# MattJBorowski1991/QuantizedMHA

Hardware: AMD Instinct MI355X
Metric: attention-fwd TFLOPS + ms/call, B16 H16 N4096 d64 (fp16 & int8) (higher is better)
Workload: dtype int8; 1 GPU; fa_tc_int8_b attention forward (BASELINE config 4); variant=fa_tc_int8_b, B_per_gpu=16, H=16, N=4096, d=64, d_model=1024, global_batch=16, parallelism=batch-shard x1 (no collective in the timed step; all-gather reported separately)

## Files before the change

quantizedmha_amd/csrc/qmha_fa_int8.hip:

```cpp
#include "qmha_common.hpp"
#include "qmha_kernels.hpp"

#include <atomic>
#include <type_traits>

namespace qmha {

static constexpr float kPtSumCap = 2047.0f / 127.0f;

template <int D>
__device__ __forceinline__ float quant_q_operand(const float* __restrict__ row, int half, v4i (&qop)[D / 32],
                                                 float slice_sc = 0.0f) {
    constexpr int KS = D / 32;
    v4f x[KS][4];
    float amax = 0.0f;
#pragma unroll
    for (int s = 0; s < KS; ++s)
#pragma unroll
        for (int c4 = 0; c4 < 4; ++c4) {
            x[s][c4] = *reinterpret_cast<const v4f*>(row + 32 * s + 16 * half + 4 * c4);
#pragma unroll
            for (int e = 0; e < 4; ++e) {
                x[s][c4][e] = nan_to_zero(x[s][c4][e]);
                amax = fmaxf(amax, fabsf(x[s][c4][e]));
            }
        }
    const float sc = slice_sc > 0.0f ? slice_sc : qmha_scale_from_absmax(wave_max64(amax));
    const float inv = 1.0f / sc;
#pragma unroll
    for (int s = 0; s < KS; ++s)
#pragma unroll
        for (int c4 = 0; c4 < 4; ++c4) {
            uint32_t w = 0;
#pragma unroll
            for (int e = 0; e < 4; ++e) w |= ((uint32_t)(uint8_t)qmha_quant_i8(x[s][c4][e], inv)) << (8 * e);
            qop[s][c4] = (int)w;
        }
    return sc;
}

__device__ PDump g_pdump;

enum { FL_MAGIC = 1, FL_LB1 = 2, FL_LB2 = 4, FL_JIT = 8, FL_LB4 = 16, FL_KFOLD = 64, FL_DUMP = 256, FL_PT = 1048576 };

template <int D, int FL>
__global__ __launch_bounds__(256, (FL & FL_LB1) ? 1 : ((FL & FL_LB2) ? 2 : 4)) void qmha_fa_int8_kernel(
    const float* __restrict__ Qf, const int8_t* __restrict__ Ki, const _Float16* __restrict__ Vh,
    const float* __restrict__ sK, const float* __restrict__ sV,
    float* __restrict__ O, int N, int H, int d_model, int nqb, float c_log2, QkDump dbg) {
    constexpr int WAVES = 4, SG = 2;
    constexpr int KS = D / 32;
    constexpr int KBYTES = SG * 32 * D;
    constexpr int VBYTES = SG * 32 * D * 2;
    constexpr int KCH = KBYTES / 16, VCH = VBYTES / 16;
    constexpr bool MAGIC = FL & FL_MAGIC;
    constexpr bool DUMP = FL & FL_DUMP;
    static_assert(D % 32 == 0 && D <= 256, "d % 32 == 0 (include/config.h:32), d <= 256 (MAGIC range)");
    static_assert(KCH % 64 == 0 && VCH % 64 == 0, "a stage is whole KiB LDS-DMA pieces");
    static_assert((KCH / SG) % 64 == 0, "a KV group is whole KiB pieces (D >= 32)");
    __shared__ __attribute__((aligned(16))) int8_t lds[2][KBYTES + VBYTES];

    const int G = N / QMHA_GROUP;
    const int wg = xcd_remap(blockIdx.x, gridDim.x);
    const int bh = wg / nqb, qb = wg % nqb;
    const int b = bh / H, k = bh % H;
    const int lane = threadIdx.x & 63;
    const int wave = __builtin_amdgcn_readfirstlane(threadIdx.x >> 6);
    const int half = lane >> 5, col = lane & 31;
    const int qg = qb * WAVES + wave;
    const bool active = qg < G;

    PDump pd{};
    if constexpr (DUMP) pd = g_pdump;
    size_t drow = 0;
    if constexpr (DUMP) drow = (size_t)bh * N + (size_t)qg * QMHA_GROUP + col;
    v4i qop[KS];
    float cq = 0.0f;
    if (active) {
        const float* qrow = Qf + ((size_t)b * N + (size_t)qg * QMHA_GROUP + col) * d_model + (size_t)k * D;
        const float sq = quant_q_operand<D>(qrow, half, qop);
        cq = sq * c_log2;
        if constexpr (DUMP) {
            int8_t* qd = dbg.Qi + ((size_t)bh * N + (size_t)qg * QMHA_GROUP + col) * D + 16 * half;
#pragma unroll
            for (int s = 0; s < KS; ++s) *reinterpret_cast<v4i*>(qd + 32 * s) = qop[s];
            if (lane == 0) dbg.sQ[(size_t)bh * G + qg] = sq;
        }
    } else {
#pragma unroll
        for (int s = 0; s < KS; ++s) qop[s] = v4i{0, 0, 0, 0};
    }
    v16f o[KS];
#pragma unroll
    for (int m = 0; m < KS; ++m) o[m] = v16f{};
    float m_run = 0.0f;
    float l_run = 0.0f;
    float anchor = 0.0f;

    const int8_t* kbase = Ki + (size_t)bh * N * D;
    const char* vbase = reinterpret_cast<const char*>(Vh + (size_t)bh * N * D);
    const float* skb = sK + (size_t)bh * G;
    const float* svb = sV + (size_t)bh * G;
    const int nst = (G + SG - 1) / SG;

    auto issue = [&](int buf, int st) {
        const int ngr = min(SG, G - st * SG);
        const int8_t* ksrc = kbase + (size_t)st * KBYTES;
        const char* vsrc = vbase + (size_t)st * VBYTES;
        int8_t* L = lds[buf];
#pragma unroll
        for (int jj = 0; jj < (KCH / 64 + WAVES - 1) / WAVES; ++jj) {
            const int inst = wave + jj * WAVES;
            if (inst < KCH / 64 && inst * 64 < ngr * (KCH / SG)) {
                const int idx = inst * 64 + lane;
                const int row = idx / (D / 16), cc = swz_src<D>(row, idx % (D / 16));
                __builtin_amdgcn_global_load_lds((gptr_t)(ksrc + row * D + 16 * cc), (lptr_t)(L + inst * 1024), 16, 0, 0);
            }
        }
#pragma unroll
        for (int jj = 0; jj < (VCH / 64 + WAVES - 1) / WAVES; ++jj) {
            const int inst = wave + jj * WAVES;
            if (inst < VCH / 64 && inst * 64 < ngr * (VCH / SG)) {
                const int idx = inst * 64 + lane;
                const int grp = idx / (4 * D), w = idx % (4 * D);
                const int d = w >> 2, cv = swz_src<64>(d, w & 3);
                __builtin_amdgcn_global_load_lds((gptr_t)(vsrc + grp * 64 * D + d * 64 + 16 * cv),
// ... 67 lines not shown
        const float e = __builtin_amdgcn_exp2f(m_new - anchor);
        l_run = fmaf(rs, e, l_run);
        m_run = m_new;
        const float scale = sp * svt * e;
#pragma unroll
        for (int m = 0; m < KS; ++m) {
            const int d = 32 * m + col;
            const int8_t* vr = L + KBYTES + gi * 64 * D + d * 64;
            v16f acc = v16f{};
#pragma unroll
            for (int ks = 0; ks < 2; ++ks) {
                const v8h vop = *reinterpret_cast<const v8h*>(vr + 16 * swz_pos<64>(d, 2 * ks + half));
                acc = __builtin_amdgcn_mfma_f32_32x32x16_f16(vop, pop[ks], acc, 0, 0, 0);
            }
            if constexpr (DUMP) {
                if (active && pd.m)
                    dump_pv_acc<false>(pd.T + (((size_t)bh * G + t) * N + qg * QMHA_GROUP + col) * D + 32 * m, acc, half);
            }
#pragma unroll
            for (int r = 0; r < 16; ++r) o[m][r] = fmaf(acc[r], scale, o[m][r]);
        }
    };

    issue(0, 0);
    qmha_dma_barrier();

    for (int st = 0; st < nst; ++st) {
        const int buf = st & 1;
        if (st + 1 < nst) issue(buf ^ 1, st + 1);
        if (active) {
            const int g0 = st * SG;
            const int ngr = min(SG, G - g0);
            const int8_t* L = lds[buf];
            if (ngr == SG) {
#pragma unroll
                for (int gi = 0; gi < SG; ++gi) tile(L, gi, g0 + gi, qk(L, gi));
            } else {
                for (int gi = 0; gi < ngr; ++gi) tile(L, gi, g0 + gi, qk(L, gi));
            }
        }
        qmha_dma_barrier();
    }

    if (active) {
        const float unanchor = __builtin_amdgcn_exp2f(anchor - m_run);
        const float l = l_run * unanchor;
        if constexpr (DUMP) {
            if (pd.m && half == 0) pd.l[drow] = l;
        }
        const bool ok = l > 1e-20f;
        float* orow = O + ((size_t)b * N + (size_t)qg * QMHA_GROUP + col) * d_model + (size_t)k * D + 4 * half;
#pragma unroll
        for (int m = 0; m < KS; ++m)
#pragma unroll
            for (int g4 = 0; g4 < 4; ++g4) {
                v4f w;
#pragma unroll
                for (int jj = 0; jj < 4; ++jj) w[jj] = ok ? (o[m][4 * g4 + jj] * unanchor) / l : 0.0f;
                *reinterpret_cast<v4f*>(orow + 32 * m + 8 * g4) = w;
            }
    }
}

__host__ __device__ constexpr int pt_slot_op(int D, int s, int j) {
    constexpr int d32[6][2] = {{0, -1}, {-1, -1}, {1, -1}, {8, -1}, {-1, -1}, {-1, -1}};
    constexpr int d64[6][2] = {{0, -1}, {2, -1}, {1, -1}, {8, -1}, {9, -1}, {3, -1}};
    constexpr int d128[6][2] = {{0, 2}, {4, 6}, {1, 3}, {8, 9}, {10, 11}, {5, 7}};
    return D == 32 ? d32[s][j] : D == 64 ? d64[s][j] : d128[s][j];
}

template <int N>
__device__ __forceinline__ void pin_regs(float (&v)[N], int lo, int hi) {
#pragma unroll
    for (int i = 0; i < N; ++i)
        if (i >= lo && i < hi) asm volatile("" : "+v"(v[i]));
}

template <int D, int WAVES, int FL>
__global__ __launch_bounds__(WAVES * 64, (FL & FL_LB2) ? 2 : ((FL & FL_LB4) ? 4 : 3)) void qmha_fa_int8_pipe_kernel(
    const float* __restrict__ Qf, const int8_t* __restrict__ Ki, const _Float16* __restrict__ Vh,
    const float* __restrict__ sK, const float* __restrict__ sV,
    float* __restrict__ O, int N, int H, int d_model, int nqb, float c_log2, QkDump dbg,
    const float* __restrict__ sQt = nullptr, int fair = 0) {
    constexpr int SG = 2, RING = 3, PF = RING - 1;
    constexpr int KBYTES = SG * 32 * D;
    constexpr int VBYTES = SG * 32 * D * 2;
    constexpr int SBYTES = KBYTES + VBYTES;
    constexpr int KCH = KBYTES / 16, VCH = VBYTES / 16;
    constexpr bool MAGIC = FL & FL_MAGIC;
    __shared__ __attribute__((aligned(16))) int8_t lds[RING][SBYTES];

    const int G = N / QMHA_GROUP;
    const int wg = xcd_remap(blockIdx.x, gridDim.x);
    const int bh = wg / nqb, qb = wg % nqb;
    const int b = bh / H, k = bh % H;
    const int lane = threadIdx.x & 63;
    const int wave = __builtin_amdgcn_readfirstlane(threadIdx.x >> 6);
    const int half = lane >> 5, col = lane & 31;
    const int qg = qb * WAVES + wave;
    const bool active = qg < G;

    v4i qop[D / 32];
    float cq = 0.0f;
    constexpr bool DUMP = FL & FL_DUMP;
    constexpr bool PT = FL & FL_PT;
    PDump pd{};
    size_t drow = 0;
    if constexpr (DUMP && !PT) {
        pd = g_pdump;
        drow = (size_t)bh * N + (size_t)qg * QMHA_GROUP + col;
    }
    auto dump_t = [&](int t, const v16f (&acc)[D / 32]) {
        if (active && pd.m) {
#pragma unroll
            for (int m = 0; m < D / 32; ++m)
                dump_pv_acc<true>(pd.T + (((size_t)bh * G + t) * N + qg * QMHA_GROUP + col) * D + 32 * m, acc[m], half);
        }
    };
    if (active) {
        const float* qrow = Qf + ((size_t)b * N + (size_t)qg * QMHA_GROUP + col) * d_model + (size_t)k * D;
        const float sq = quant_q_operand<D>(qrow, half, qop, PT ? sQt[bh] : 0.0f);
        cq = sq * c_log2;
        if constexpr (DUMP) {
            int8_t* qd = dbg.Qi + ((size_t)bh * N + (size_t)qg * QMHA_GROUP + col) * D + 16 * half;
#pragma unroll
            for (int s = 0; s < D / 32; ++s) *reinterpret_cast<v4i*>(qd + 32 * s) = qop[s];
            if (lane == 0) dbg.sQ[(size_t)bh * G + qg] = sq;
        }
    } else {
#pragma unroll
        for (int ks = 0; ks < D / 32; ++ks) qop[ks] = v4i{0, 0, 0, 0};
    }
    const int8_t* kbase = Ki + (size_t)bh * N * D;
    const char* vbase = reinterpret_cast<const char*>(Vh) + (size_t)bh * N * D * 2;
    const int sstride = PT ? 1 : G;
    const float* skb = sK + (size_t)bh * sstride;
    const float* svb = sV + (size_t)bh * sstride;
    const int nst = (G + SG - 1) / SG;

    constexpr int KJ = (KCH / 64 + WAVES - 1) / WAVES, VJ = (VCH / 64 + WAVES - 1) / WAVES;
    constexpr bool SPREAD = WAVES >= KCH / 64 + VCH / 64;
    const int vw = SPREAD ? (wave + WAVES - KCH / 64) % WAVES : wave;
    int koff[KJ], voff[VJ];
#pragma unroll
    for (int jj = 0; jj < KJ; ++jj) {
        const int idx = (wave + jj * WAVES) * 64 + lane;
        const int row = idx / (D / 16), cc = swz_src<D>(row, idx % (D / 16));
        koff[jj] = row * D + 16 * cc;
    }
#pragma unroll
    for (int jj = 0; jj < VJ; ++jj) {
        const int idx = (vw + jj * WAVES) * 64 + lane;
        const int grp = idx / (4 * D), w = idx % (4 * D);
        const int d = w >> 2, cv = swz_src<64>(d, w & 3);
        voff[jj] = grp * 64 * D + d * 64 + 16 * cv;
    }
    auto issue_at = [&](int st, int slot) {
        const int ngr = min(SG, G - st * SG);
        int8_t* L = lds[slot];
#pragma unroll
        for (int jj = 0; jj < KJ; ++jj) {
            const int inst = wave + jj * WAVES;
            if (inst < KCH / 64 && inst * 64 < ngr * (KCH / SG))
                buffer_load_lds16(kbase, N * D, (lptr_t)(L + inst * 1024), koff[jj], st * KBYTES);
        }
#pragma unroll
        for (int jj = 0; jj < VJ; ++jj) {
            const int inst = vw + jj * WAVES;
            if (inst < VCH / 64 && inst * 64 < ngr * (VCH / SG))
                buffer_load_lds16(vbase, N * D * 2, (lptr_t)(L + KBYTES + inst * 1024), voff[jj], st * VBYTES);
        }
    };
    auto issue = [&](int st) { issue_at(st, st % RING); };
    auto kop_at = [&](int slot, int par, int ks) {
        const int8_t* L = lds[slot];
        const int krow = par * 32 + col;
        return *reinterpret_cast<const v4i*>(L + krow * D + 16 * swz_pos<D>(krow, 2 * ks + half));
    };
    auto vop_at = [&](int slot, int par, int m, int ks) {
        const int8_t* L = lds[slot];
        const int d = 32 * m + col;
        return *reinterpret_cast<const v8h*>(L + KBYTES + par * 64 * D + d * 64 + 16 * swz_pos<64>(d, 2 * ks + half));
    };
    auto kop_of = [&](int t, int ks) { return kop_at((t >> 1) % RING, t & 1, ks); };
    auto vop_of = [&](int t, int m, int ks) { return vop_at((t >> 1) % RING, t & 1, m, ks); };

    v16i magic_blk;
#pragma unroll
    for (int r = 0; r < 16; ++r) magic_blk[r] = MAGIC ? 0x4B400000 : 0;
    if constexpr (MAGIC) asm volatile("" : "+v"(magic_blk));

    constexpr int MB = D / 32;
    constexpr int KS = D / 32;
    constexpr int NOPS = 2 * MB + KS;
    constexpr int kSlot64[6] = {1, 1, 1, 1, 1, 1};
    constexpr int kOps64[6] = {0, 2, 1, 1000, 3, 1001};
    constexpr int kSlot32[6] = {1, 0, 1, 1, 0, 0};
    constexpr int kOps32[3] = {0, 1, 1000};
    constexpr int kSlot128[6] = {2, 2, 2, 2, 2, 2};
    constexpr int kOps128[12] = {0, 2, 4, 1000, 6, 1, 1001, 3, 5, 1002, 7, 1003};
    auto slot_n = [&](int c) { return D == 32 ? kSlot32[c] : (D == 64 ? kSlot64[c] : kSlot128[c]); };
    auto op_at = [&](int i) { return D == 32 ? kOps32[i] : (D == 64 ? kOps64[i] : kOps128[i]); };
    static_assert(D == 32 || D == 64 || D == 128, "pipelined kernel: d in {32, 64, 128}");
    static_assert(NOPS == (D == 32 ? 3 : (D == 64 ? 6 : 12)), "MFMA schedule table");

    v16f o[MB];
#pragma unroll
    for (int m = 0; m < MB; ++m) o[m] = v16f{};
    float m_run = 0.0f;
    float l_run = 0.0f;
    float anchor = 0.0f;
    v16i s_cur, s_nxt;
    auto qk = [&](const v4i& kk, int ks) {
        s_nxt = __builtin_amdgcn_mfma_i32_32x32x32_i8(kk, qop[ks], ks == 0 ? magic_blk : s_nxt, 0, 0, 0);
    };
    v8h pc[2], pp[2];
    float scale_prev = 0.0f;
    v16f a[MB];
    constexpr bool JIT = FL & FL_JIT;
    constexpr bool KFOLD = MAGIC && (FL & FL_KFOLD);
    static_assert(KFOLD, "the pipelined kernel ships with FL_MAGIC | FL_KFOLD");
    float h_c = 0.0f, h_m = 0.0f, h_k = 0.0f, h_f = 1.0f, h_sp = 0.0f, h_invp = 0.0f, h_cap = 0.0f;
    const float c_pt = PT ? __int_as_float((__float_as_int(cq * skb[0]) + 2) & ~3) : 0.0f;
    auto head = [&](const v16i& s, int t) {
        float c = PT ? c_pt : cq * skb[t];
        const int mxi = half_swap_max_i(tree_max16_i(s));
        if constexpr (!PT) c = __int_as_float((__float_as_int(c) + 2) & ~3);
        const float sfmax = __int_as_float(mxi) - QMHA_MAGIC_RNE;
        const float xm = sfmax * c;
        h_m = fmaxf(m_run, xm);
        h_k = fmaf(c, QMHA_MAGIC_RNE, h_m);
        const float delta = fmaf(c, -QMHA_MAGIC_RNE, h_k) - h_m;
        h_f = fmaf(delta, 0.69314718055994531f, 1.0f);
        const float xmax = fmaf(sfmax, c, -h_m);
        h_c = c;
        const float pmax = half_max32_nonneg(__builtin_amdgcn_exp2f(xmax));
        const float sp = fmaxf(pmax, 1.27e-6f) * (1.0f / 127.0f);
        h_invp = __builtin_amdgcn_rcpf(sp);
        h_invp *= h_f;
        h_sp = sp * 16777216.0f;
    };

    auto pt_base = [&](float mb) {
        h_m = mb;
        h_k = fmaf(c_pt, QMHA_MAGIC_RNE, mb);
        const float delta = fmaf(c_pt, -QMHA_MAGIC_RNE, h_k) - mb;
        h_f = fmaf(delta, 0.69314718055994531f, 1.0f);
        h_invp = 127.0f * h_f;
        h_cap = kPtSumCap / h_f;
    };
    auto pt_rowmax = [&](const v16i& s) {
        return (__int_as_float(half_swap_max_i(tree_max16_i(s))) - QMHA_MAGIC_RNE) * c_pt;
    };
    if constexpr (PT) pt_base(0.0f);
    issue(0);
    if (nst > 1) issue(1);
    qmha_dma_barrier();
#pragma unroll
    for (int ks = 0; ks < KS; ++ks) qk(kop_of(0, ks), ks);
    s_cur = s_nxt;

#define QMHA_FENCE() __builtin_amdgcn_sched_barrier(0)
    auto iter = [&](int t, auto HP, auto HN, auto PH) {
        constexpr bool has_prev = decltype(HP)::value, has_next = decltype(HN)::value;
        constexpr int ph = decltype(PH)::value;
        const int odd = ph >= 0 ? ((1 + ph) & 1) : (t & 1);
        const int slot_p = ph >= 0 ? ((ph >> 1) % RING) : (((t - 1) >> 1) % RING);
        const int par_p = ph >= 0 ? (ph & 1) : ((t - 1) & 1);
        const int slot_nx = ph >= 0 ? (((2 + ph) >> 1) % RING) : (((t + 1) >> 1) % RING);
        const int par_n = ph >= 0 ? (ph & 1) : ((t + 1) & 1);
        auto vop = [&](int m, int ks) { return vop_at(slot_p, par_p, m, ks); };
        auto kop = [&](int ks) { return kop_at(slot_nx, par_n, ks); };
        const int dma_st = (t >> 1) + PF;
        const int dma_slot = ph >= 0 ? ((((1 + ph) >> 1) + PF) % RING) : (((t >> 1) + PF) % RING);
        if (odd) {
            qmha_dma_barrier();
            if (dma_st < nst) issue_at(dma_st, dma_slot);
        }
        if constexpr (DUMP) {
            if (active) {
                int32_t* sd = dbg.S + ((size_t)bh * N + (size_t)qg * QMHA_GROUP + col) * N + (size_t)t * QMHA_GROUP;
#pragma unroll
                for (int r = 0; r < 16; ++r) sd[acc_row(r, half)] = s_cur[r] - 0x4B400000;
            }
        }
        v8h vv[MB][2];
        v4i kk[KS];
        if constexpr (has_prev && !JIT) {
#pragma unroll
            for (int ks = 0; ks < 2; ++ks)
#pragma unroll
                for (int m = 0; m < MB; ++m) vv[m][ks] = vop(m, ks);
        }
        if constexpr (has_next && !JIT) {
#pragma unroll
            for (int ks = 0; ks < KS; ++ks) kk[ks] = kop(ks);
        }
        QMHA_FENCE();
        int op_i = 0;
        auto mfmas = [&](int c) {
#pragma unroll
            for (int j = 0; j < 2; ++j) {
                if (j < slot_n(c)) {
                    const int op = op_at(op_i++);
                    if (op >= 1000) {
                        const int ks = op - 1000;
                        if (has_next) qk(JIT ? kop(ks) : kk[ks], ks);
                    } else {
                        const int m = op >> 1, ks = op & 1;
                        if (has_prev)
                            a[m] = __builtin_amdgcn_mfma_f32_32x32x16_f16(JIT ? vop(m, ks) : vv[m][ks], pp[ks],
                                                                          ks == 0 ? v16f{} : a[m], 0, 0, 0);
                    }
                }
            }
        };
        head(s_cur, t);
        QMHA_FENCE();
        const float c = h_c, m_new = h_m, kn = h_k;
        if (__builtin_amdgcn_ballot_w64(m_new - anchor > 48.0f)) {
            const float f = __builtin_amdgcn_exp2f(anchor - m_new);
#pragma unroll
            for (int m = 0; m < MB; ++m) o[m] *= f;
            l_run *= f;
            scale_prev *= f;
            anchor = m_new;
        }
        mfmas(0);
        QMHA_FENCE();
        const float sp = h_sp, invp = h_invp;
        const float e = __builtin_amdgcn_exp2f(m_new - anchor);
        float x[16];
#pragma unroll
        for (int r = 0; r < 8; ++r) x[r] = fmaf(__int_as_float(s_cur[r]), c, -kn);
        QMHA_FENCE();
        mfmas(1);
        QMHA_FENCE();
#pragma unroll
        for (int r = 8; r < 16; ++r) x[r] = fmaf(__int_as_float(s_cur[r]), c, -kn);
        QMHA_FENCE();
        mfmas(2);
        QMHA_FENCE();
        float p[16];
#pragma unroll
        for (int r = 0; r < 8; ++r) p[r] = __builtin_amdgcn_exp2f(x[r]);
        QMHA_FENCE();
        mfmas(3);
        QMHA_FENCE();
#pragma unroll
        for (int r = 8; r < 16; ++r) p[r] = __builtin_amdgcn_exp2f(x[r]);
        QMHA_FENCE();
        mfmas(4);
        QMHA_FENCE();
#pragma unroll
        for (int r = 0; r < 8; ++r) {
            const float t0 = fmaf(p[2 * r], invp, QMHA_MAGIC_RNE), t1 = fmaf(p[2 * r + 1], invp, QMHA_MAGIC_RNE);
            const v2h h2 = __builtin_bit_cast(v2h, __builtin_amdgcn_perm(__float_as_uint(t1), __float_as_uint(t0), 0x05040100u));
            pc[r >> 2][2 * (r & 3)] = h2[0];
            pc[r >> 2][2 * (r & 3) + 1] = h2[1];
        }
        if constexpr (DUMP) {
            if (active && pd.m) {
                if (half == 0) pd.m[drow * G + t] = m_new;
                if (lane == 0) pd.sP[((size_t)bh * G + qg) * G + t] = sp * (1.0f / 16777216.0f);
                dump_p_operand<true>(pd.Pi + drow * N + (size_t)t * QMHA_GROUP, pc, half);
            }
        }
        QMHA_FENCE();
        mfmas(5);
        QMHA_FENCE();
        const float rs = tree_sum16(p);
        l_run = fmaf(rs, e * h_f, l_run);
        m_run = m_new;
        const float scale_t = sp * svb[t] * e;
        if constexpr (has_prev) {
            if constexpr (DUMP) dump_t(t - 1, a);
#pragma unroll
            for (int m = 0; m < MB; ++m)
#pragma unroll
                for (int r = 0; r < 16; ++r) o[m][r] = fmaf(a[m][r], scale_prev, o[m][r]);
        }
        QMHA_FENCE();
        pp[0] = pc[0];
        pp[1] = pc[1];
        scale_prev = scale_t;
        if constexpr (has_next) s_cur = s_nxt;
    };
    float alpha_prev = 1.0f;
    bool rescale_prev = false;
    auto iter_pt = [&](int t, auto HP, auto HN, auto PH) {
        constexpr bool has_prev = decltype(HP)::value, has_next = decltype(HN)::value;
        constexpr int ph = decltype(PH)::value;
        const int odd = ph >= 0 ? ((1 + ph) & 1) : (t & 1);
        const int slot_p = ph >= 0 ? ((ph >> 1) % RING) : (((t - 1) >> 1) % RING);
        const int par_p = ph >= 0 ? (ph & 1) : ((t - 1) & 1);
        const int slot_nx = ph >= 0 ? (((2 + ph) >> 1) % RING) : (((t + 1) >> 1) % RING);
        const int par_n = ph >= 0 ? (ph & 1) : ((t + 1) & 1);
        const int dma_st = (t >> 1) + PF;
        const int dma_slot = ph >= 0 ? ((((1 + ph) >> 1) + PF) % RING) : (((t >> 1) + PF) % RING);
        if (odd) {
            qmha_dma_barrier();
            if (dma_st < nst) issue_at(dma_st, dma_slot);
        }
        if constexpr (DUMP) {
            if (active) {
                int32_t* sd = dbg.S + ((size_t)bh * N + (size_t)qg * QMHA_GROUP + col) * N + (size_t)t * QMHA_GROUP;
#pragma unroll
                for (int r = 0; r < 16; ++r) sd[acc_row(r, half)] = s_cur[r] - 0x4B400000;
            }
        }
        v8h vv[MB][2];
        v4i kk[KS];
        auto rd_slot = [&](int s) {
#pragma unroll
            for (int j = 0; j < 2; ++j) {
                const int op = pt_slot_op(D, s, j);
                if (op >= 0 && op < 8) {
                    if constexpr (has_prev)
                        if ((op >> 1) < MB) vv[(op >> 1) % MB][op & 1] = vop_at(slot_p, par_p, op >> 1, op & 1);
                } else if (op >= 8) {
                    if constexpr (has_next)
                        if (op - 8 < KS) kk[(op - 8) % KS] = kop_at(slot_nx, par_n, op - 8);
                }
            }
        };
        auto mf_slot = [&](int s) {
#pragma unroll
            for (int j = 0; j < 2; ++j) {
                const int op = pt_slot_op(D, s, j);
                if (op >= 0 && op < 8) {
                    if constexpr (has_prev) {
                        const int m = (op >> 1) % MB;
                        if ((op >> 1) < MB) o[m] = __builtin_amdgcn_mfma_f32_32x32x16_f16(vv[m][op & 1], pp[op & 1], o[m], 0, 0, 0);
                    }
                } else if (op >= 8) {
                    if constexpr (has_next)
                        if (op - 8 < KS) qk(kk[(op - 8) % KS], op - 8);
                }
            }
        };
        float x[16], p[16], q[16];
        auto exps = [&](int r0, int r1) {
#pragma unroll
            for (int r = 0; r < 16; ++r)
                if (r >= r0 && r < r1) p[r] = __builtin_amdgcn_exp2f(x[r]);
        };
        auto quant = [&](int r0, int r1) {
#pragma unroll
            for (int r = 0; r < 16; ++r)
                if (r >= r0 && r < r1) q[r] = fmaf(p[r], h_invp, QMHA_MAGIC_RNE);
        };
        auto perms = [&](int j0, int j1) {
#pragma unroll
            for (int j = 0; j < 8; ++j)
                if (j >= j0 && j < j1) {
                    const v2h h2 = __builtin_bit_cast(v2h, __builtin_amdgcn_perm(__float_as_uint(q[2 * j + 1]),
                                                                               __float_as_uint(q[2 * j]), 0x05040100u));
// ... 45 lines not shown
        QMHA_FENCE();
        mf_slot(2);
        QMHA_FENCE();
        exps(8, 12);
        perms(2, 4);
        QMHA_FENCE();
        rd_slot(4);
        quant(8, 12);
        float rs2 = (p[8] + p[9]) + (p[10] + p[11]);
        asm volatile("" : "+v"(rs2));
        QMHA_FENCE();
        mf_slot(3);
        QMHA_FENCE();
        exps(12, 16);
        perms(4, 6);
        QMHA_FENCE();
        rd_slot(5);
        quant(12, 16);
        float rs3 = (p[12] + p[13]) + (p[14] + p[15]);
        asm volatile("" : "+v"(rs3));
        QMHA_FENCE();
        mf_slot(4);
        QMHA_FENCE();
        perms(6, 8);
        QMHA_FENCE();
        float ts = (rs0 + rs1) + (rs2 + rs3);
        float alpha_t = 1.0f;
        bool rescale_t = false;
        if constexpr (has_prev) {
            const uint64_t over = __builtin_amdgcn_ballot_w64(ts > h_cap);
            if (over) {
                rescale_t = true;
                const float xm = pt_rowmax(s_cur);
                const uint32_t rows = (uint32_t)over | (uint32_t)(over >> 32);
                const float mb = ((rows >> col) & 1u) ? xm : m_run;
                alpha_t = __builtin_amdgcn_exp2f(m_run - mb);
                l_run *= alpha_t;
                pt_base(mb);
                m_run = mb;
#pragma unroll
                for (int r = 0; r < 16; ++r) x[r] = fmaf(__int_as_float(s_cur[r]), c_pt, -h_k);
                exps(0, 16);
                quant(0, 16);
                perms(0, 8);
                ts = tree_sum16(p);
            }
        }
        l_run = fmaf(ts, h_f, l_run);
        QMHA_FENCE();
        mf_slot(5);
        QMHA_FENCE();
        pp[0] = pc[0];
        pp[1] = pc[1];
        alpha_prev = alpha_t;
        rescale_prev = rescale_t;
        if constexpr (has_next) s_cur = s_nxt;
    };
    auto run_iter = [&](int t, auto HP, auto HN, auto PH) {
        if constexpr (PT)
            iter_pt(t, HP, HN, PH);
        else
            iter(t, HP, HN, PH);
    };
    using T1 = std::integral_constant<bool, true>;
    using F0 = std::integral_constant<bool, false>;
    using DYN = std::integral_constant<int, -1>;
    if (PT && G == 1) {
        if constexpr (PT) run_iter(0, F0{}, F0{}, DYN{});
    } else {
        auto set_prio = [&](int tt) {
            const int q = (4 * tt) / G;
            if (q <= 0)
                __builtin_amdgcn_s_setprio(3);
            else if (q == 1)
                __builtin_amdgcn_s_setprio(2);
            else if (q == 2)
                __builtin_amdgcn_s_setprio(1);
            else
                __builtin_amdgcn_s_setprio(0);
        };
        if (fair) set_prio(0);
        run_iter(0, F0{}, T1{}, DYN{});
        int t = 1;
        constexpr int PER = 2 * RING;
        for (; t + PER <= G - 1; t += PER) {
            if (fair) set_prio(t);
            run_iter(t, T1{}, T1{}, std::integral_constant<int, 0>{});
            run_iter(t + 1, T1{}, T1{}, std::integral_constant<int, 1>{});
            run_iter(t + 2, T1{}, T1{}, std::integral_constant<int, 2>{});
            run_iter(t + 3, T1{}, T1{}, std::integral_constant<int, 3>{});
            run_iter(t + 4, T1{}, T1{}, std::integral_constant<int, 4>{});
            run_iter(t + 5, T1{}, T1{}, std::integral_constant<int, 5>{});
        }
        for (; t < G - 1; ++t) run_iter(t, T1{}, T1{}, DYN{});
        run_iter(G - 1, T1{}, F0{}, DYN{});
    }
#undef QMHA_FENCE
    {
        const int t = G - 1;
        if constexpr (PT) {
            if (rescale_prev) {
#pragma unroll
                for (int m = 0; m < MB; ++m) o[m] *= alpha_prev;
            }
#pragma unroll
            for (int ks = 0; ks < 2; ++ks)
#pragma unroll
                for (int m = 0; m < MB; ++m)
                    o[m] = __builtin_amdgcn_mfma_f32_32x32x16_f16(vop_of(t, m, ks), pp[ks], o[m], 0, 0, 0);
        } else {
#pragma unroll
            for (int ks = 0; ks < 2; ++ks)
#pragma unroll
                for (int m = 0; m < MB; ++m)
                    a[m] = __builtin_amdgcn_mfma_f32_32x32x16_f16(vop_of(t, m, ks), pp[ks], ks == 0 ? v16f{} : a[m], 0, 0, 0);
            if constexpr (DUMP) dump_t(t, a);
#pragma unroll
            for (int m = 0; m < MB; ++m) o[m] += a[m] * scale_prev;
        }
    }
    if (active) {
        const float unanchor = PT ? 16777216.0f * (svb[0] / 127.0f) : __builtin_amdgcn_exp2f(anchor - m_run);
        const float l = PT ? half_swap_add(l_run) : half_swap_add(l_run) * unanchor;
        if constexpr (DUMP && !PT) {
            if (pd.m && half == 0) pd.l[drow] = l;
        }
        const bool ok = l > 1e-20f;
        float* orow = O + ((size_t)b * N + (size_t)qg * QMHA_GROUP + col) * d_model + (size_t)k * D + 4 * half;
#pragma unroll
        for (int m = 0; m < MB; ++m)
#pragma unroll
            for (int g4 = 0; g4 < 4; ++g4) {
                v4f w;
#pragma unroll
                for (int jj = 0; jj < 4; ++jj) w[jj] = ok ? (o[m][4 * g4 + jj] * unanchor) / l : 0.0f;
                *reinterpret_cast<v4f*>(orow + 32 * m + 8 * g4) = w;
            }
    }
}

template <int D>
__global__ __launch_bounds__(64) void qmha_debug_qk_int32_kernel(const int8_t* __restrict__ Qi, const int8_t* __restrict__ Ki,
                                                                int N, int bh, int32_t* __restrict__ S) {
    constexpr int KS = D / 32;
    const int qg = blockIdx.x, kg = blockIdx.y;
    const int lane = threadIdx.x, half = lane >> 5, col = lane & 31;
    const int8_t* qp = Qi + ((size_t)bh * N + (size_t)qg * 32 + col) * D + 16 * half;
    const int8_t* kp = Ki + ((size_t)bh * N + (size_t)kg * 32 + col) * D + 16 * half;
    v16i s = {};
#pragma unroll
    for (int ks = 0; ks < KS; ++ks)
        s = __builtin_amdgcn_mfma_i32_32x32x32_i8(*reinterpret_cast<const v4i*>(kp + 32 * ks),
                                                  *reinterpret_cast<const v4i*>(qp + 32 * ks), s, 0, 0, 0);
#pragma unroll
    for (int r = 0; r < 16; ++r) S[((size_t)qg * 32 + col) * N + (size_t)kg * 32 + acc_row(r, half)] = s[r];
}

template <int D, int FL>
static hipError_t fa_int8_launch(const Int8Workspace& w, const float* Qf, float* O, int B, int N, int H, int d_model,
                                 hipStream_t stream, QkDump dbg = QkDump{}) {
    const int G = N / QMHA_GROUP;
    const int nqb = (G + 3) / 4;
    const float c_log2 = softmax_scale_log2(D);
    hipLaunchKernelGGL((qmha_fa_int8_kernel<D, FL>), dim3(B * H * nqb), dim3(256), 0, stream, Qf, w.Ki, w.Vh, w.sK, w.sV,
                       O, N, H, d_model, nqb, c_log2, dbg);
    return hipGetLastError();
}

template <int D, int WAVES, int FL>
static long long pipe_slots() {
    static std::atomic<long long> slots_of[64];
    int dev = 0;
    if (hipGetDevice(&dev) != hipSuccess || dev < 0 || dev >= 64) return 0;
    long long slots = slots_of[dev].load(std::memory_order_relaxed);
    if (slots <= 0) {
// ... 213 lines not shown
                    pt_base(qb, mb);
                    softmax_p(qb);
                }
            }
        }
#pragma unroll
        for (int qb = 0; qb < 2; ++qb) {
            l_run[qb] = fmaf(ts[qb], h_f[qb], l_run[qb]);
            v4i pw;
#pragma unroll
            for (int i = 0; i < 4; ++i)
                pw[i] = (int)__builtin_amdgcn_perm(__float_as_uint(q[qb][2 * i + 1]), __float_as_uint(q[qb][2 * i]), 0x05040100u);
            const v8h pop = __builtin_bit_cast(v8h, pw);
#pragma unroll
            for (int m = 0; m < DB; ++m) o[m][qb] = __builtin_amdgcn_mfma_f32_16x16x32_f16(vop[m], pop, o[m][qb], 0, 0, 0);
        }
    };

    issue(0, 0);
    qmha_dma_barrier();
    int t = 0;
    auto stage = [&](auto BUF, int st) {
        constexpr int buf = decltype(BUF)::value;
        if (st + 1 < nst) issue(buf ^ 1, st + 1);
        if (active) {
            const char* L = lds[buf];
            const int ngr = G - st * SG;
#pragma unroll
            for (int gi = 0; gi < SG; ++gi) {
                if (gi == 0 || gi < ngr) tile(L, gi, qk(L, gi), t == 0, st * SG + gi);
                ++t;
                __builtin_amdgcn_sched_barrier(0);
            }
        }
        qmha_dma_barrier();
    };
    int st = 0;
    for (; st + 2 <= nst; st += 2) {
        stage(std::integral_constant<int, 0>{}, st);
        stage(std::integral_constant<int, 1>{}, st + 1);
    }
    if (st < nst) stage(std::integral_constant<int, 0>{}, st);
    if (active) {
        const float unanchor = 16777216.0f * (sV[bh] / 127.0f);
#pragma unroll
        for (int qb = 0; qb < 2; ++qb) {
            float l = l_run[qb];
            l += __shfl_xor(l, 16);
            l += __shfl_xor(l, 32);
            const bool ok = l > 1e-20f;
            float* orow = O + ((size_t)b * N + (size_t)qg * QMHA_GROUP + 16 * qb + r16) * d_model + (size_t)k * D + 4 * grp;
#pragma unroll
            for (int m = 0; m < DB; ++m) {
                v4f w;
#pragma unroll
                for (int j = 0; j < 4; ++j) w[j] = ok ? (o[m][qb][j] * unanchor) / l : 0.0f;
                *reinterpret_cast<v4f*>(orow + 16 * m) = w;
            }
        }
    }
}

template <int D, int FL, int WAVES = 4>
static hipError_t fa_int8_pt_launch(const Int8Workspace& w, const float* Qf, float* O, int B, int N, int H, int d_model,
                                    hipStream_t stream, QkDump dbg = QkDump{}) {
    const int G = N / QMHA_GROUP;
    const int nqb = (G + WAVES - 1) / WAVES;
    const float c_log2 = softmax_scale_log2(D);
    const int rounds = pipe_rounds<D, WAVES, FL | FL_PT>((long long)B * H * nqb);
    const int fair = rounds > 0 && rounds <= kFairMaxRounds;
    hipLaunchKernelGGL((qmha_fa_int8_pipe_kernel<D, WAVES, FL | FL_PT>), dim3(B * H * nqb), dim3(WAVES * 64), 0, stream,
                       Qf, w.Ki, w.Vh, w.sK, w.sV, O, N, H, d_model, nqb, c_log2, dbg, (const float*)w.sQ, fair);
    return hipGetLastError();
}

constexpr int kD64Flags = FL_MAGIC | FL_KFOLD, kD32Flags = FL_MAGIC | FL_KFOLD;
constexpr int kD128Flags = FL_MAGIC | FL_KFOLD | FL_JIT | FL_LB2, kPtD32Extra = FL_LB4;
template <int D>
constexpr int kAnyFlags = FL_MAGIC | (D > 128 ? FL_LB1 : FL_LB2);

template <int D, int XFL = 0>
static hipError_t fa_int8_d(const Int8Workspace& w, const float* Qf, float* O, int B, int N, int H, int d_model,
                            hipStream_t stream, QkDump dbg = QkDump{}) {
    if constexpr (D == 32) return fa_int8_pipe_launch<D, 4, kD32Flags | XFL>(w, Qf, O, B, N, H, d_model, stream, dbg);
    else if constexpr (D == 64) return fa_int8_pipe_launch<D, 4, kD64Flags | XFL>(w, Qf, O, B, N, H, d_model, stream, dbg);
    else if constexpr (D == 128) return fa_int8_pipe_launch<D, 4, kD128Flags | XFL>(w, Qf, O, B, N, H, d_model, stream, dbg);
    else return fa_int8_launch<D, kAnyFlags<D> | XFL>(w, Qf, O, B, N, H, d_model, stream, dbg);
}

static long long device_cus() {
    static std::atomic<int> cus_of[64];
    int dev = 0;
    if (hipGetDevice(&dev) != hipSuccess || dev < 0 || dev >= 64) return 0;
    int c = cus_of[dev].load(std::memory_order_relaxed);
    if (c <= 0) {
        if (hipDeviceGetAttribute(&c, hipDeviceAttributeMultiprocessorCount, dev) != hipSuccess || c <= 0) return 0;
        cus_of[dev].store(c, std::memory_order_relaxed);
    }
    return c;
}

template <int D, int WAVES, bool DUMP = false>
static hipError_t fa_int8_pt_v3_launch(const Int8Workspace& w, const float* Qf, float* O, int B, int N, int H, int d_model,
                                       hipStream_t stream, QkDump dbg = QkDump{}) {
    const int G = N / QMHA_GROUP;
    const int nqb = (G + WAVES - 1) / WAVES;
    const float c_log2 = softmax_scale_log2(D);
    hipLaunchKernelGGL((qmha_fa_int8_pt_v3_kernel<D, WAVES, 2, DUMP>), dim3(B * H * nqb), dim3(WAVES * 64), 0, stream, Qf,
                       w.Ki, w.Vh, w.sQ, w.sK, w.sV, O, N, H, d_model, nqb, c_log2, dbg);
    return hipGetLastError();
}

hipError_t launch_fa_int8_pt_main(const Int8Workspace& w, const float* Qf, float* O, int B, int N, int H, int D,
                                  int d_model, hipStream_t stream) {
    switch (D) {
        case 32: return fa_int8_pt_launch<32, kD32Flags | kPtD32Extra>(w, Qf, O, B, N, H, d_model, stream);
        case 64: {
            const long long wgs8 = (long long)B * H * ((N / QMHA_GROUP + 7) / 8), cus = device_cus();
            if (cus > 0 && wgs8 <= cus) return fa_int8_pt_v3_launch<64, 4>(w, Qf, O, B, N, H, d_model, stream);
            return fa_int8_pt_v3_launch<64, 8>(w, Qf, O, B, N, H, d_model, stream);
        }
        case 128: return fa_int8_pt_launch<128, kD128Flags>(w, Qf, O, B, N, H, d_model, stream);
        default: return hipErrorInvalidValue;
    }
}

#define QMHA_INT8_D_CASES(X) X(32) X(64) X(96) X(128) X(160) X(192) X(224) X(256)

hipError_t launch_fa_int8_main(const Int8Workspace& w, const float* Qf, float* O, int B, int N, int H, int D,
                               int d_model, hipStream_t stream) {
    switch (D) {
#define QMHA_CASE(d) \
    case d: return fa_int8_d<d>(w, Qf, O, B, N, H, d_model, stream);
        QMHA_INT8_D_CASES(QMHA_CASE)
#undef QMHA_CASE
        default: return hipErrorInvalidValue;
    }
}

hipError_t launch_fa_int8_dump(const Int8Workspace& w, const float* Qf, float* O, int B, int N, int H, int D,
                               int d_model, QkDump dbg, hipStream_t stream) {
    if ((D == 32 || D == 64 || D == 128) && N / QMHA_GROUP < 2) return hipErrorInvalidValue;
    switch (D) {
#define QMHA_CASE(d) \
    case d: return fa_int8_d<d, FL_DUMP>(w, Qf, O, B, N, H, d_model, stream, dbg);
        QMHA_INT8_D_CASES(QMHA_CASE)
#undef QMHA_CASE
        default: return hipErrorInvalidValue;
    }
}

hipError_t launch_fa_int8_pstage_dump(const Int8Workspace& w, const float* Qf, float* O, int B, int N, int H, int D,
                                      int d_model, QkDump dbg, PDump pd) {
    hipError_t e = hipMemcpyToSymbol(HIP_SYMBOL(g_pdump), &pd, sizeof(pd));
    if (e != hipSuccess) return e;
    if ((D == 32 || D == 64 || D == 128) && N / QMHA_GROUP < 2) {
        switch (D) {
            case 32: e = fa_int8_launch<32, FL_DUMP>(w, Qf, O, B, N, H, d_model, nullptr, dbg); break;
            case 64: e = fa_int8_launch<64, FL_DUMP>(w, Qf, O, B, N, H, d_model, nullptr, dbg); break;
            default: e = fa_int8_launch<128, FL_DUMP>(w, Qf, O, B, N, H, d_model, nullptr, dbg); break;
        }
    } else {
        e = launch_fa_int8_dump(w, Qf, O, B, N, H, D, d_model, dbg, nullptr);
    }
    const PDump none{};
    const hipError_t e2 = hipMemcpyToSymbol(HIP_SYMBOL(g_pdump), &none, sizeof(none));
// ... 29 lines not shown
```

Baseline: 753.7 TFLOPS.

## Widen int8 pipe stages to four KV groups with staggered K ring and scalar tile scales

For D<=64 in the non-PT int8 pipelined kernel, each LDS stage now holds four KV groups instead of two, using a two-slot ring. K loads are shifted two groups ahead of V, and the prologue preloads the extra K groups. The goal is to cut the number of DMA barriers and syncthreads per group. Per-tile sK/sV scales are now loaded once per barrier as vectors into scalar registers, replacing a global load in every iteration. An ablation env switch is added behind a compile flag; the trade-off is more complex slot and parity indexing and a shallower ring.

```diff
diff --git a/quantizedmha_amd/csrc/qmha_fa_int8.hip b/quantizedmha_amd/csrc/qmha_fa_int8.hip
--- a/quantizedmha_amd/csrc/qmha_fa_int8.hip
+++ b/quantizedmha_amd/csrc/qmha_fa_int8.hip
@@ -2,6 +2,7 @@
 #include "qmha_kernels.hpp"
 
 #include <atomic>
+#include <cstdlib>
 #include <type_traits>
 
 namespace qmha {
@@ -41,7 +42,8 @@
 
 __device__ PDump g_pdump;
 
-enum { FL_MAGIC = 1, FL_LB1 = 2, FL_LB2 = 4, FL_JIT = 8, FL_LB4 = 16, FL_KFOLD = 64, FL_DUMP = 256, FL_PT = 1048576 };
+enum { FL_MAGIC = 1, FL_LB1 = 2, FL_LB2 = 4, FL_JIT = 8, FL_LB4 = 16, FL_KFOLD = 64, FL_DUMP = 256,
+       FL_ABL_STAGE2 = 512, FL_ABL_TILESCALE = 1024, FL_PT = 1048576 };
 
 template <int D, int FL>
 __global__ __launch_bounds__(256, (FL & FL_LB1) ? 1 : ((FL & FL_LB2) ? 2 : 4)) void qmha_fa_int8_kernel(
@@ -275,12 +277,15 @@
     const float* __restrict__ sK, const float* __restrict__ sV,
     float* __restrict__ O, int N, int H, int d_model, int nqb, float c_log2, QkDump dbg,
     const float* __restrict__ sQt = nullptr, int fair = 0) {
-    constexpr int SG = 2, RING = 3, PF = RING - 1;
+    constexpr bool S4 = !(FL & FL_PT) && D <= 64 && !(FL & FL_ABL_STAGE2);
+    constexpr int SG = S4 ? 4 : 2, LSG = S4 ? 2 : 1, RING = S4 ? 2 : 3, PF = RING - 1;
+    constexpr int KSH = S4 ? 2 : 0;
     constexpr int KBYTES = SG * 32 * D;
     constexpr int VBYTES = SG * 32 * D * 2;
     constexpr int SBYTES = KBYTES + VBYTES;
     constexpr int KCH = KBYTES / 16, VCH = VBYTES / 16;
     constexpr bool MAGIC = FL & FL_MAGIC;
+    constexpr bool STSC = !(FL & FL_PT) && !(FL & FL_ABL_TILESCALE);
     __shared__ __attribute__((aligned(16))) int8_t lds[RING][SBYTES];
 
     const int G = N / QMHA_GROUP;
@@ -334,37 +339,52 @@
     constexpr int KJ = (KCH / 64 + WAVES - 1) / WAVES, VJ = (VCH / 64 + WAVES - 1) / WAVES;
     constexpr bool SPREAD = WAVES >= KCH / 64 + VCH / 64;
     const int vw = SPREAD ? (wave + WAVES - KCH / 64) % WAVES : wave;
-    int koff[KJ], voff[VJ];
-#pragma unroll
-    for (int jj = 0; jj < KJ; ++jj) {
+    static_assert(!S4 || (WAVES * 1024 / D) % 16 == 0, "a wave's K pieces share one swizzle phase");
+    constexpr int KR = S4 ? 1 : KJ, VR = S4 ? 1 : VJ;
+    int koff[KR], voff[VR];
+#pragma unroll
+    for (int jj = 0; jj < KR; ++jj) {
         const int idx = (wave + jj * WAVES) * 64 + lane;
         const int row = idx / (D / 16), cc = swz_src<D>(row, idx % (D / 16));
         koff[jj] = row * D + 16 * cc;
     }
 #pragma unroll
-    for (int jj = 0; jj < VJ; ++jj) {
+    for (int jj = 0; jj < VR; ++jj) {
         const int idx = (vw + jj * WAVES) * 64 + lane;
         const int grp = idx / (4 * D), w = idx % (4 * D);
         const int d = w >> 2, cv = swz_src<64>(d, w & 3);
         voff[jj] = grp * 64 * D + d * 64 + 16 * cv;
     }
     auto issue_at = [&](int st, int slot) {
-        const int ngr = min(SG, G - st * SG);
+        const int ngr = min(SG, G - st * SG), ngk = min(SG, G - st * SG - KSH);
         int8_t* L = lds[slot];
 #pragma unroll
         for (int jj = 0; jj < KJ; ++jj) {
             const int inst = wave + jj * WAVES;
-            if (inst < KCH / 64 && inst * 64 < ngr * (KCH / SG))
-                buffer_load_lds16(kbase, N * D, (lptr_t)(L + inst * 1024), koff[jj], st * KBYTES);
+            if (inst < KCH / 64 && inst * 64 < ngk * (KCH / SG))
+                buffer_load_lds16(kbase, N * D, (lptr_t)(L + inst * 1024), koff[S4 ? 0 : jj],
+                                  st * KBYTES + KSH * 32 * D + (S4 ? jj * WAVES * 1024 : 0));
         }
 #pragma unroll
         for (int jj = 0; jj < VJ; ++jj) {
             const int inst = vw + jj * WAVES;
             if (inst < VCH / 64 && inst * 64 < ngr * (VCH / SG))
-                buffer_load_lds16(vbase, N * D * 2, (lptr_t)(L + KBYTES + inst * 1024), voff[jj], st * VBYTES);
+                buffer_load_lds16(vbase, N * D * 2, (lptr_t)(L + KBYTES + inst * 1024), voff[S4 ? 0 : jj],
+                                  st * VBYTES + (S4 ? jj * WAVES * 1024 : 0));
         }
     };
     auto issue = [&](int st) { issue_at(st, st % RING); };
+    auto issue_k01 = [&]() {
+        int8_t* L = lds[1];
+#pragma unroll
+        for (int jj = 0; jj < KJ; ++jj) {
+            const int inst = wave + jj * WAVES;
+            if (inst < KCH / 64 && inst * 64 >= KSH * (KCH / SG))
+                buffer_load_lds16(kbase, N * D, (lptr_t)(L + inst * 1024), koff[0] + (jj * WAVES * 1024 - KSH * 32 * D), 0);
+        }
+    };
+    auto kslot_of = [&](int t) { return RING == 2 ? (((t - KSH) >> LSG) & 1) : (((t - KSH) >> LSG) % RING); };
+    auto vslot_of = [&](int t) { return RING == 2 ? ((t >> LSG) & 1) : ((t >> LSG) % RING); };
     auto kop_at = [&](int slot, int par, int ks) {
         const int8_t* L = lds[slot];
         const int krow = par * 32 + col;
@@ -375,8 +395,8 @@
         const int d = 32 * m + col;
         return *reinterpret_cast<const v8h*>(L + KBYTES + par * 64 * D + d * 64 + 16 * swz_pos<64>(d, 2 * ks + half));
     };
-    auto kop_of = [&](int t, int ks) { return kop_at((t >> 1) % RING, t & 1, ks); };
-    auto vop_of = [&](int t, int m, int ks) { return vop_at((t >> 1) % RING, t & 1, m, ks); };
+    auto kop_of = [&](int t, int ks) { return kop_at(kslot_of(t), (t - KSH) & (SG - 1), ks); };
+    auto vop_of = [&](int t, int m, int ks) { return vop_at(vslot_of(t), t & (SG - 1), m, ks); };
 
     v16i magic_blk;
 #pragma unroll
@@ -415,8 +435,8 @@
     static_assert(KFOLD, "the pipelined kernel ships with FL_MAGIC | FL_KFOLD");
     float h_c = 0.0f, h_m = 0.0f, h_k = 0.0f, h_f = 1.0f, h_sp = 0.0f, h_invp = 0.0f, h_cap = 0.0f;
     const float c_pt = PT ? __int_as_float((__float_as_int(cq * skb[0]) + 2) & ~3) : 0.0f;
-    auto head = [&](const v16i& s, int t) {
-        float c = PT ? c_pt : cq * skb[t];
+    auto head = [&](const v16i& s, float skt) {
+        float c = PT ? c_pt : cq * skt;
         const int mxi = half_swap_max_i(tree_max16_i(s));
         if constexpr (!PT) c = __int_as_float((__float_as_int(c) + 2) & ~3);
         const float sfmax = __int_as_float(mxi) - QMHA_MAGIC_RNE;
@@ -447,28 +467,54 @@
     };
     if constexpr (PT) pt_base(0.0f);
     issue(0);
-    if (nst > 1) issue(1);
+    if constexpr (S4)
+        issue_k01();
+    else if (nst > 1)
+        issue(1);
     qmha_dma_barrier();
 #pragma unroll
     for (int ks = 0; ks < KS; ++ks) qk(kop_of(0, ks), ks);
     s_cur = s_nxt;
 
 #define QMHA_FENCE() __builtin_amdgcn_sched_barrier(0)
+    float st_sk[SG], st_sv[SG];
+#pragma unroll
+    for (int i = 0; i < SG; ++i) st_sk[i] = st_sv[i] = 0.0f;
     auto iter = [&](int t, auto HP, auto HN, auto PH) {
         constexpr bool has_prev = decltype(HP)::value, has_next = decltype(HN)::value;
         constexpr int ph = decltype(PH)::value;
-        const int odd = ph >= 0 ? ((1 + ph) & 1) : (t & 1);
-        const int slot_p = ph >= 0 ? ((ph >> 1) % RING) : (((t - 1) >> 1) % RING);
-        const int par_p = ph >= 0 ? (ph & 1) : ((t - 1) & 1);
-        const int slot_nx = ph >= 0 ? (((2 + ph) >> 1) % RING) : (((t + 1) >> 1) % RING);
-        const int par_n = ph >= 0 ? (ph & 1) : ((t + 1) & 1);
+        const int bar = ph >= 0 ? (ph % SG == 0) : ((t & (SG - 1)) == 1);
+        const int slot_p = ph >= 0 ? ((ph >> LSG) % RING) : vslot_of(t - 1);
+        const int par_p = ph >= 0 ? (ph & (SG - 1)) : ((t - 1) & (SG - 1));
+        const int slot_nx = ph >= 0 ? (((2 + ph - KSH) >> LSG) % RING) : kslot_of(t + 1);
+        const int par_n = ph >= 0 ? ((2 + ph - KSH) & (SG - 1)) : ((t + 1 - KSH) & (SG - 1));
         auto vop = [&](int m, int ks) { return vop_at(slot_p, par_p, m, ks); };
         auto kop = [&](int ks) { return kop_at(slot_nx, par_n, ks); };
-        const int dma_st = (t >> 1) + PF;
-        const int dma_slot = ph >= 0 ? ((((1 + ph) >> 1) + PF) % RING) : (((t >> 1) + PF) % RING);
-        if (odd) {
-            qmha_dma_barrier();
+        const int dma_st = ((t - 1) >> LSG) + PF;
+        const int dma_slot = ph >= 0 ? (((ph >> LSG) + PF) % RING) : ((((t - 1) >> LSG) + PF) % RING);
+        constexpr bool stsc = STSC && ph >= 0;
+        float skt = 0.0f, svt = 0.0f;
+        if (bar) {
+            if constexpr (stsc) {
+                typedef float vsg_t __attribute__((ext_vector_type(SG), aligned(4)));
+                const vsg_t lk = *reinterpret_cast<const vsg_t*>(skb + t), lv = *reinterpret_cast<const vsg_t*>(svb + t);
+                QMHA_FENCE();
+                __builtin_amdgcn_s_waitcnt(0x0070);
+#pragma unroll
+                for (int i = 0; i < SG; ++i) {
+                    st_sk[i] = lk[i];
+                    st_sv[i] = lv[i];
+                    asm volatile("" : "+s"(st_sk[i]), "+s"(st_sv[i]));
+                }
+                __syncthreads();
+            } else {
+                qmha_dma_barrier();
+            }
             if (dma_st < nst) issue_at(dma_st, dma_slot);
+        }
+        if constexpr (stsc) {
+            skt = st_sk[ph & (SG - 1)];
+            svt = st_sv[ph & (SG - 1)];
         }
         if constexpr (DUMP) {
             if (active) {
@@ -508,7 +554,7 @@
                 }
             }
         };
-        head(s_cur, t);
+        head(s_cur, stsc ? skt : skb[t]);
         QMHA_FENCE();
         const float c = h_c, m_new = h_m, kn = h_k;
         if (__builtin_amdgcn_ballot_w64(m_new - anchor > 48.0f)) {
@@ -565,7 +611,7 @@
         const float rs = tree_sum16(p);
         l_run = fmaf(rs, e * h_f, l_run);
         m_run = m_new;
-        const float scale_t = sp * svb[t] * e;
+        const float scale_t = sp * (stsc ? svt : svb[t]) * e;
         if constexpr (has_prev) {
             if constexpr (DUMP) dump_t(t - 1, a);
 #pragma unroll
@@ -777,7 +823,7 @@
         if (fair) set_prio(0);
         run_iter(0, F0{}, T1{}, DYN{});
         int t = 1;
-        constexpr int PER = 2 * RING;
+        constexpr int PER = SG * RING;
         for (; t + PER <= G - 1; t += PER) {
             if (fair) set_prio(t);
             run_iter(t, T1{}, T1{}, std::integral_constant<int, 0>{});
@@ -786,6 +832,10 @@
             run_iter(t + 3, T1{}, T1{}, std::integral_constant<int, 3>{});
             run_iter(t + 4, T1{}, T1{}, std::integral_constant<int, 4>{});
             run_iter(t + 5, T1{}, T1{}, std::integral_constant<int, 5>{});
+            if constexpr (PER == 8) {
+                run_iter(t + 6, T1{}, T1{}, std::integral_constant<int, 6>{});
+                run_iter(t + 7, T1{}, T1{}, std::integral_constant<int, 7>{});
+            }
         }
         for (; t < G - 1; ++t) run_iter(t, T1{}, T1{}, DYN{});
         run_iter(G - 1, T1{}, F0{}, DYN{});
@@ -1165,6 +1215,16 @@
 template <int D, int XFL = 0>
 static hipError_t fa_int8_d(const Int8Workspace& w, const float* Qf, float* O, int B, int N, int H, int d_model,
                             hipStream_t stream, QkDump dbg = QkDump{}) {
+#ifdef QMHA_ABLATION
+    if constexpr ((D == 32 || D == 64) && XFL == 0) {
+        static const int abl = [] { const char* e = getenv("QMHA_INT8_ABL"); return e ? atoi(e) : 0; }();
+        constexpr int fl = D == 32 ? kD32Flags : kD64Flags;
+        if (abl == 1) return fa_int8_pipe_launch<D, 4, fl | FL_ABL_STAGE2>(w, Qf, O, B, N, H, d_model, stream, dbg);
+        if (abl == 2) return fa_int8_pipe_launch<D, 4, fl | FL_ABL_TILESCALE>(w, Qf, O, B, N, H, d_model, stream, dbg);
+        if (abl == 3)
+            return fa_int8_pipe_launch<D, 4, fl | FL_ABL_STAGE2 | FL_ABL_TILESCALE>(w, Qf, O, B, N, H, d_model, stream, dbg);
+    }
+#endif
     if constexpr (D == 32) return fa_int8_pipe_launch<D, 4, kD32Flags | XFL>(w, Qf, O, B, N, H, d_model, stream, dbg);
     else if constexpr (D == 64) return fa_int8_pipe_launch<D, 4, kD64Flags | XFL>(w, Qf, O, B, N, H, d_model, stream, dbg);
     else if constexpr (D == 128) return fa_int8_pipe_launch<D, 4, kD128Flags | XFL>(w, Qf, O, B, N, H, d_model, stream, dbg);
```

Result: no change. 759.0 TFLOPS (median of 6 runs) (+0.7%).
